# tanwanirahul/surreal

Hardware: AMD Instinct MI355X
Metric: PPO learner env-steps/sec/node (GAE+update) at 1/2/4/8 GPUs; % HBM roofline (higher is better)
Workload: dtype f32; 1 GPU; C3: synthetic PPO learner batch, reference PPO defaults (LSTM 100, horizon 5, heads 300x200, n_step 25, adapt, z-filter, 10/10 epochs), SawyerLift state dims (obs 42, act 8), 1024 segments split over 1 GPU(s) (1024 per GPU); segments_per_gpu=1024, n_step=25, env_steps_per_learn_per_gpu=25600, global_segments=1024, parallelism=single, epochs_run_last=10, ppo_mode=adapt, launch=hipGraph replay

## Files before the change

surreal_amd/csrc/lstm_mfma.hip:

```cpp
#include "smi_device.hpp"
#include "smi_internal.hpp"
#include "lstm_cell.hpp"

namespace smi {

constexpr int LR = 16;
#ifdef SMI_PROF
__device__ unsigned long long g_lstm_ticks[8];
#endif

__host__ __device__ inline int lstm_ld(int k) {
  int l = round4(k);
  if ((l & 7) != 4) l += 4;
  return l;
}

__host__ __device__ inline int lstm_q(int K) { return (((K + 3) >> 2) + 3) & ~3; }

constexpr int MAXUT = 4;
__global__ void __launch_bounds__(kWG)
lstm_fwd_kernel(LstmFwdArgs a) {
  if (a.skip && a.skip[0] != 0) return;
  const int keepS = a.keep > 0 ? a.keep : a.S;
  extern __shared__ __attribute__((aligned(16))) float sm[];
  const int H = a.H, B = a.B, G4 = 4 * H;
  const int LDH = lstm_ld(4 * lstm_q(H));
  float* hA[2] = {sm, sm + LR * LDH};
  const int lane = threadIdx.x & 63, wave = threadIdx.x >> 6;
  const int li = lane & 15, lk = lane >> 4;
  const int r0 = blockIdx.x * LR;
  const int NUT = (H + 15) >> 4;
  const int64_t BH = (int64_t)B * H;
  for (int e = threadIdx.x; e < LR * LDH; e += kWG) {
    const int r = e / LDH, k = e - r * LDH;
    const bool ok = k < H && r0 + r < B;
    const float v = ok ? a.h0[(int64_t)(r0 + r) * H + k] : 0.f;
    hA[0][e] = v;
    hA[1][e] = 0.f;
    if (ok) a.hbuf[(int64_t)(r0 + r) * H + k] = v;
  }
  float creg[MAXUT][4];
#pragma unroll
  for (int u = 0; u < MAXUT; ++u) {
    const int unit = (wave + 4 * u) * 16 + li;
#pragma unroll
    for (int i = 0; i < 4; ++i) {
      const int gr = r0 + lk * 4 + i;
      const bool ok = unit < H && gr < B;
      creg[u][i] = ok ? a.c0[(int64_t)gr * H + unit] : 0.f;
      if (ok && a.cbuf) a.cbuf[(int64_t)gr * H + unit] = creg[u][i];
    }
  }
  const float* wrow[MAXUT][4];
  float bh[MAXUT][4];
#pragma unroll
  for (int u = 0; u < MAXUT; ++u) {
    int unit = (wave + 4 * u) * 16 + li;
    unit = unit < H ? unit : H - 1;
#pragma unroll
    for (int g = 0; g < 4; ++g) {
      wrow[u][g] = a.w_hh + (int64_t)(g * H + unit) * H;
      bh[u][g] = a.b_hh[g * H + unit];
    }
  }
  const int nks = (H + 3) >> 2;
  __syncthreads();
  for (int t = 0; t < a.S; ++t) {
    const float* hp = hA[t & 1];
    float* hn = hA[(t + 1) & 1];
    float xp[MAXUT][4][4];
#pragma unroll
    for (int u = 0; u < MAXUT; ++u) {
      int unit = (wave + 4 * u) * 16 + li;
      unit = unit < H ? unit : H - 1;
#pragma unroll
      for (int i = 0; i < 4; ++i) {
        int gr = r0 + lk * 4 + i;
        gr = gr < B ? gr : B - 1;
        const float* xr = a.xproj + ((int64_t)t * B + gr) * G4 + unit;
#pragma unroll
        for (int g = 0; g < 4; ++g) xp[u][g][i] = xr[g * H];
      }
    }
    f32x4 acc[MAXUT][4];
#pragma unroll
    for (int u = 0; u < MAXUT; ++u)
#pragma unroll
      for (int g = 0; g < 4; ++g) acc[u][g] = f32x4{0.f, 0.f, 0.f, 0.f};
    const float* ap = hp + li * LDH + lk;
    int ks = 0;
    for (; ks + 4 <= nks; ks += 4) {
      float av[4], bv[MAXUT][4][4];
#pragma unroll
      for (int s = 0; s < 4; ++s) {
        const int k = (ks + s) * 4 + lk;
        const int kc = k < H ? k : H - 1;
        av[s] = ap[(ks + s) * 4];
#pragma unroll
        for (int u = 0; u < MAXUT; ++u)
#pragma unroll
          for (int g = 0; g < 4; ++g) bv[u][g][s] = wrow[u][g][kc];
      }
#pragma unroll
      for (int s = 0; s < 4; ++s)
#pragma unroll
        for (int u = 0; u < MAXUT; ++u)
#pragma unroll
          for (int g = 0; g < 4; ++g) acc[u][g] = mfma4(av[s], bv[u][g][s], acc[u][g]);
    }
    for (; ks < nks; ++ks) {
      const int k = ks * 4 + lk;
      const int kc = k < H ? k : H - 1;
      const float av = ap[ks * 4];
#pragma unroll
      for (int u = 0; u < MAXUT; ++u)
#pragma unroll
        for (int g = 0; g < 4; ++g) acc[u][g] = mfma4(av, wrow[u][g][kc], acc[u][g]);
    }
#pragma unroll
    for (int u = 0; u < MAXUT; ++u) {
      const int ut = wave + 4 * u;
      const int unit = ut * 16 + li;
      if (ut >= NUT) continue;
#pragma unroll
      for (int i = 0; i < 4; ++i) {
        const int row = lk * 4 + i, gr = r0 + row;
        const float gi = xp[u][0][i] + (acc[u][0][i] + bh[u][0]);
        const float gf = xp[u][1][i] + (acc[u][1][i] + bh[u][1]);
        const float gg = xp[u][2][i] + (acc[u][2][i] + bh[u][2]);
        const float go = xp[u][3][i] + (acc[u][3][i] + bh[u][3]);
        const float ig = sigm(gi), fg = sigm(gf), cg = ftanh(gg), og = sigm(go);
        const float c = fg * creg[u][i] + ig * cg;
        const float h = og * ftanh(c);
        const bool ok = unit < H && gr < B;
        creg[u][i] = ok ? c : 0.f;
        if (unit < H) hn[row * LDH + unit] = ok ? h : 0.f;
        if (ok) {
          a.hbuf[(int64_t)(t + 1) * BH + (int64_t)gr * H + unit] = h;
          if (a.cbuf && t < keepS) a.cbuf[(int64_t)(t + 1) * BH + (int64_t)gr * H + unit] = c;
          if (a.gates && t < keepS) {
            float* gp = a.gates + ((int64_t)t * B + gr) * G4 + unit;
            gp[0] = ig; gp[H] = fg; gp[2 * H] = cg; gp[3 * H] = og;
          }
        }
      }
    }
    __syncthreads();
  }
}



__global__ void __launch_bounds__(kWG)
lstm_bwd_kernel(LstmBwdArgs a) {
  if (a.skip && a.skip[0] != 0) return;
  extern __shared__ __attribute__((aligned(16))) float sm[];
  const int H = a.H, B = a.B, G4 = 4 * H;
  const int LDG = lstm_ld(G4);
  float* dG[2] = {sm, sm + LR * LDG};
  const int lane = threadIdx.x & 63, wave = threadIdx.x >> 6;
  const int li = lane & 15, lk = lane >> 4;
  const int r0 = blockIdx.x * LR;
  const int NUT = (H + 15) >> 4;
  const int64_t BH = (int64_t)B * H;
  for (int e = threadIdx.x; e < 2 * LR * LDG; e += kWG) sm[e] = 0.f;
  float dcreg[MAXUT][4];
  f32x4 dhrec[MAXUT];
#pragma unroll
  for (int u = 0; u < MAXUT; ++u) {
    dhrec[u] = f32x4{0.f, 0.f, 0.f, 0.f};
#pragma unroll
    for (int i = 0; i < 4; ++i) dcreg[u][i] = 0.f;
  }
  int ucl[MAXUT];
#pragma unroll
  for (int u = 0; u < MAXUT; ++u) {
    const int unit = (wave + 4 * u) * 16 + li;
    ucl[u] = unit < H ? unit : H - 1;
  }
  const int nks = G4 >> 2;
  __syncthreads();
  for (int t = a.S - 1; t >= 0; --t) {
    float* dg = dG[t & 1];
#pragma unroll
    for (int u = 0; u < MAXUT; ++u) {
      const int ut = wave + 4 * u;
      const int unit = ut * 16 + li;
      if (ut >= NUT) continue;
#pragma unroll
      for (int i = 0; i < 4; ++i) {
        const int row = lk * 4 + i;
        int gr = r0 + row;
        const bool ok = unit < H && gr < B;
        gr = gr < B ? gr : B - 1;
        const int uc = ucl[u];
        const float* gp = a.gates + ((int64_t)t * B + gr) * G4 + uc;
        const float ig = gp[0], fg = gp[H], cg = gp[2 * H], og = gp[3 * H];
        const float c = a.cbuf[(int64_t)(t + 1) * BH + (int64_t)gr * H + uc];
        const float cp = a.cbuf[(int64_t)t * BH + (int64_t)gr * H + uc];
        const float dh = a.dh[(int64_t)t * BH + (int64_t)gr * H + uc] + dhrec[u][i];
        const float tc = ftanh(c);
        const float dc = dh * og * (1.f - tc * tc) + dcreg[u][i];
        const float d_o = (dh * tc) * (og * (1.f - og));
        const float d_i = (dc * cg) * (ig * (1.f - ig));
        const float d_g = (dc * ig) * (1.f - cg * cg);
        const float d_f = (dc * cp) * (fg * (1.f - fg));
        dcreg[u][i] = ok ? dc * fg : 0.f;
        if (ok) {
          float* o = a.dgates + ((int64_t)t * B + gr) * G4 + unit;
          o[0] = d_i; o[H] = d_f; o[2 * H] = d_g; o[3 * H] = d_o;
          float* l = dg + row * LDG + unit;
          l[0] = d_i; l[H] = d_f; l[2 * H] = d_g; l[3 * H] = d_o;
        }
      }
    }
    __syncthreads();
    if (t == 0) break;
#pragma unroll
    for (int u = 0; u < MAXUT; ++u) dhrec[u] = f32x4{0.f, 0.f, 0.f, 0.f};
    const float* ap = dg + li * LDG + lk;
    int ks = 0;
    for (; ks + 8 <= nks; ks += 8) {
      float av[8], bv[MAXUT][8];
#pragma unroll
      for (int s = 0; s < 8; ++s) {
        const int k = (ks + s) * 4 + lk;
        av[s] = ap[(ks + s) * 4];
#pragma unroll
        for (int u = 0; u < MAXUT; ++u) bv[u][s] = a.w_hh[(int64_t)k * H + ucl[u]];
      }
#pragma unroll
      for (int s = 0; s < 8; ++s)
#pragma unroll
        for (int u = 0; u < MAXUT; ++u) dhrec[u] = mfma4(av[s], bv[u][s], dhrec[u]);
    }
    for (; ks < nks; ++ks) {
      const int k = ks * 4 + lk;
      const float av = ap[ks * 4];
#pragma unroll
      for (int u = 0; u < MAXUT; ++u) dhrec[u] = mfma4(av, a.w_hh[(int64_t)k * H + ucl[u]], dhrec[u]);
    }
  }
}

constexpr int kWG8 = 512;
template <int N>
__device__ __forceinline__ void load_row(const float* r, int n, float* dst) {
  static_assert(N % 4 == 0, "rows in float4 runs");
  const uintptr_t ad = reinterpret_cast<uintptr_t>(r);
  if ((ad & 15) == 0 && (n & 3) == 0) {
#pragma unroll
    for (int k = 0; k < N; k += 4) {
      const float4 v = k < n ? *reinterpret_cast<const float4*>(r + k) : float4{0.f, 0.f, 0.f, 0.f};
      dst[k] = v.x; dst[k + 1] = v.y; dst[k + 2] = v.z; dst[k + 3] = v.w;
    }
  } else if ((ad & 7) == 0 && (n & 1) == 0) {
#pragma unroll
    for (int k = 0; k < N; k += 2) {
      const float2 v = k < n ? *reinterpret_cast<const float2*>(r + k) : float2{0.f, 0.f};
      dst[k] = v.x; dst[k + 1] = v.y;
    }
  } else {
#pragma unroll
    for (int k = 0; k < N; ++k) dst[k] = k < n ? r[k] : 0.f;
  }
}

constexpr int LR4 = 4;
constexpr int LSTM_HQ = 4;

__device__ __forceinline__ f32x4 mfma4x64(float a, float b, f32x4 c) {
  return __builtin_amdgcn_mfma_f32_4x4x1f32(a, b, c, 4, 0, 0);
}

__device__ __attribute__((aligned(16))) float g_lstm_zero4[4] = {0.f, 0.f, 0.f, 0.f};
template <int N, int V>
__device__ __forceinline__ void load_row_v(const float* r, int n, float* dst) {
  static_assert(N % 4 == 0 && (V == 4 || V == 2), "vector rows");
#pragma unroll
  for (int k = 0; k < N; k += V) {
    const float* src = k < n ? r + k : g_lstm_zero4;
    if constexpr (V == 4) {
      const float4 v = *reinterpret_cast<const float4*>(src);
      dst[k] = v.x; dst[k + 1] = v.y; dst[k + 2] = v.z; dst[k + 3] = v.w;
    } else {
      const float2 v = *reinterpret_cast<const float2*>(src);
      dst[k] = v.x; dst[k + 1] = v.y;
    }
  }
}

template <int N>
__device__ __forceinline__ void load_col(const float* t, int n, int ld, uint32_t zoff, int col,
                                         float* dst) {
#pragma unroll
  for (int k = 0; k < N; ++k) {
    const uint32_t row = k < n ? (uint32_t)(k * ld) : zoff;
    dst[k] = t[row + (uint32_t)col];
  }
}

template <int KP, int KX, bool VF = false, bool IMG = false>
__global__ void __launch_bounds__(kWG8)
lstm_fwd_r4_kernel(LstmFwdArgs a) {
  if (a.skip && a.skip[0] != 0) return;
  LSTM_T0();
  const int keepS = a.keep > 0 ? a.keep : a.S;
  constexpr int KXS = KX > 0 ? KX : 8;
  __shared__ __attribute__((aligned(16))) float hS[2][LR4 * KP];
  __shared__ __attribute__((aligned(16))) float xS[2][LR4 * KXS];
  __shared__ float pre[LR4][4 * KP];
  const int H = a.H, B = a.B, G4 = 4 * H;
  const int tid = threadIdx.x, lane = tid & 63, wave = tid >> 6;
  const int r0 = blockIdx.x * LR4;
  const int64_t BH = (int64_t)B * H;
  const int col = wave * 64 + lane;
  const bool cact = wave * 64 < G4;
  const int colc = col < G4 ? col : G4 - 1;
  float w[KP];
  float wx[KXS];
  float bh = a.b_hh[colc];
  if constexpr (KX > 0) bh += a.b_ih[colc];
  if constexpr (IMG) {
    load_col<KP>(a.w_hh, H, G4, (uint32_t)(H * G4), colc, w);
    if constexpr (KX > 0) load_col<KX>(a.w_ih, a.din, G4, (uint32_t)((a.din + H) * G4), colc, wx);
  } else if constexpr (VF) {
    load_row_v<KP, 4>(a.w_hh + (int64_t)colc * H, H, w);
    if constexpr (KX > 0) load_row_v<KX, 2>(a.w_ih + (int64_t)colc * a.din, a.din, wx);
  } else {
    load_row<KP>(a.w_hh + (int64_t)colc * H, H, w);
    if constexpr (KX > 0) load_row<KX>(a.w_ih + (int64_t)colc * a.din, a.din, wx);
  }
  const int xr = tid / KXS, xk = tid - (tid / KXS) * KXS;
  const bool xown = KX > 0 && tid < LR4 * KXS;
  const int64_t xoff0 = (int64_t)min(r0 + xr, B - 1) * a.ldx + min(xk, a.din - 1);
  const bool xval = xk < a.din;
  auto xload = [&](int t) -> float { return a.x[(int64_t)t * B * a.ldx + xoff0]; };
  float xnext = 0.f, x0 = 0.f;
  if constexpr (KX > 0) {
    x0 = xload(0);
    xnext = xload(a.S > 1 ? 1 : 0);
  }
  const bool cell = tid < LR4 * H;
  const int crow = cell ? tid / H : 0;
  const int cunit = cell ? tid - crow * H : 0;
  const int cgr = r0 + crow;
  const bool cok = cell && cgr < B;
  const float c0v = a.c0[(int64_t)min(cgr, B - 1) * H + cunit];
  static_assert(LR4 * KP <= kWG8, "one h0 slot per thread");
  const int he = min(tid, LR4 * KP - 1);
  const int hr = he / KP, hk = he - hr * KP;
  float h0v = a.h0[(int64_t)min(r0 + hr, B - 1) * H + min(hk, H - 1)];
  asm volatile("" : "+v"(h0v));
  if constexpr (KX > 0) asm volatile("" : "+v"(x0));
  if constexpr (KX > 0) {
    if (xown && a.S > 0) xS[0][xr * KXS + xk] = xval ? x0 : 0.f;
  }
  float creg = cok ? c0v : 0.f;
  if (cok && a.cbuf) a.cbuf[(int64_t)cgr * H + cunit] = creg;
  if (tid < LR4 * KP) {
    const bool ok = hk < H && r0 + hr < B;
    const float v = ok ? h0v : 0.f;
    hS[0][he] = v;
    hS[1][he] = 0.f;
    if (ok) a.hbuf[(int64_t)(r0 + hr) * H + hk] = v;
  }
  int64_t xoff[4];
#pragma unroll
  for (int i = 0; i < 4; ++i) {
    const int gr = r0 + i < B ? r0 + i : B - 1;
    xoff[i] = (int64_t)gr * G4 + colc;
  }
  float xp[4] = {0.f, 0.f, 0.f, 0.f};
  if (KX == 0 && a.S > 0) {
#pragma unroll
    for (int i = 0; i < 4; ++i) xp[i] = a.xproj[xoff[i]];
  }
  __syncthreads();
  LSTM_TICK(6);
  f32x4 acc[8];
#pragma unroll
  for (int j = 0; j < 8; ++j) acc[j] = f32x4{0.f, 0.f, 0.f, 0.f};
  auto x_part = [&](int tt) {
    if constexpr (KX > 0) {
      const float4* xr4 = reinterpret_cast<const float4*>(xS[tt & 1] + (lane & 3) * KXS);
      constexpr int NQX = KX / 4;
      float4 q[LSTM_HQ];
#pragma unroll
      for (int j = 0; j < LSTM_HQ && j < NQX; ++j) q[j] = xr4[j];
#pragma unroll
      for (int j = 0; j < NQX; ++j) {
        const float4 u = q[j % LSTM_HQ];
        const int ab = (j & 1) * 4;
        acc[ab + 0] = mfma4x64(u.x, wx[4 * j + 0], acc[ab + 0]);
        acc[ab + 1] = mfma4x64(u.y, wx[4 * j + 1], acc[ab + 1]);
        acc[ab + 2] = mfma4x64(u.z, wx[4 * j + 2], acc[ab + 2]);
        acc[ab + 3] = mfma4x64(u.w, wx[4 * j + 3], acc[ab + 3]);
        if (j + LSTM_HQ < NQX) q[j % LSTM_HQ] = xr4[j + LSTM_HQ];
      }
      __builtin_amdgcn_sched_group_barrier(0x100, LSTM_HQ < NQX ? LSTM_HQ : NQX, 0);
#pragma unroll
      for (int j = 0; j < NQX; ++j) {
        __builtin_amdgcn_sched_group_barrier(0x008, 4, 0);
        if (j + LSTM_HQ < NQX) __builtin_amdgcn_sched_group_barrier(0x100, 1, 0);
      }
    }
  };
  if (cact && a.S > 0) x_part(0);
  for (int t = 0; t < a.S; ++t) {
    const float* hp = hS[t & 1];
    float* hn = hS[(t + 1) & 1];
    if (cact) {
      const float4* hr = reinterpret_cast<const float4*>(hp + (lane & 3) * KP);
      constexpr int NQ = KP / 4;
      float4 q[LSTM_HQ];
#pragma unroll
      for (int j = 0; j < LSTM_HQ; ++j) q[j] = hr[j];
#pragma unroll
      for (int j = 0; j < NQ; ++j) {
        const float4 u = q[j % LSTM_HQ];
        const int ab = (j & 1) * 4;
        acc[ab + 0] = mfma4x64(u.x, w[4 * j + 0], acc[ab + 0]);
        acc[ab + 1] = mfma4x64(u.y, w[4 * j + 1], acc[ab + 1]);
        acc[ab + 2] = mfma4x64(u.z, w[4 * j + 2], acc[ab + 2]);
        acc[ab + 3] = mfma4x64(u.w, w[4 * j + 3], acc[ab + 3]);
        if (j + LSTM_HQ < NQ) q[j % LSTM_HQ] = hr[j + LSTM_HQ];
      }
      __builtin_amdgcn_sched_group_barrier(0x100, LSTM_HQ, 0);
#pragma unroll
      for (int j = 0; j < NQ; ++j) {
        __builtin_amdgcn_sched_group_barrier(0x008, 4, 0);
        if (j + LSTM_HQ < NQ) __builtin_amdgcn_sched_group_barrier(0x100, 1, 0);
      }
      const f32x4 sum = ((acc[0] + acc[1]) + (acc[2] + acc[3])) +
                        ((acc[4] + acc[5]) + (acc[6] + acc[7]));
      if (col < G4) {
#pragma unroll
        for (int i = 0; i < 4; ++i) pre[i][col] = xp[i] + (sum[i] + bh);
      }
      if (KX == 0 && t + 1 < a.S) {
#pragma unroll
        for (int i = 0; i < 4; ++i) xp[i] = a.xproj[(int64_t)(t + 1) * B * G4 + xoff[i]];
      }
    }
    if constexpr (KX > 0) {
      if (xown && t + 1 < a.S) xS[(t + 1) & 1][xr * KXS + xk] = xval ? xnext : 0.f;
      if (xown && t + 2 < a.S) xnext = xload(t + 2);
    }
    LSTM_TICK(0);
    __syncthreads();
    if (cact) {
#pragma unroll
      for (int j = 0; j < 8; ++j) acc[j] = f32x4{0.f, 0.f, 0.f, 0.f};
      if (t + 1 < a.S) x_part(t + 1);
    }
    if (cell) {
      const float ig = sigm(pre[crow][cunit]), fg = sigm(pre[crow][H + cunit]);
      const float cg = ftanh(pre[crow][2 * H + cunit]), og = sigm(pre[crow][3 * H + cunit]);
      const float c = fg * creg + ig * cg;
      const float h = og * ftanh(c);
      creg = cok ? c : 0.f;
      hn[crow * KP + cunit] = cok ? h : 0.f;
      if (cok) {
        a.hbuf[(int64_t)(t + 1) * BH + (int64_t)cgr * H + cunit] = h;
        if (a.cbuf && t < keepS) a.cbuf[(int64_t)(t + 1) * BH + (int64_t)cgr * H + cunit] = c;
        if (a.gates && t < keepS) {
          float* gp = a.gates + ((int64_t)t * B + cgr) * G4 + cunit;
          gp[0] = ig; gp[H] = fg; gp[2 * H] = cg; gp[3 * H] = og;
        }
      }
    }
    LSTM_TICK(1);
    __syncthreads();
    LSTM_TICK(2);
  }
}

template <int KW>
__global__ void __launch_bounds__(kWG8)
lstm_bwd_r4_kernel(LstmBwdArgs a) {
  if (a.skip && a.skip[0] != 0) return;
  LSTM_T0();
  constexpr int G4P = 4 * 128 + KW;
  __shared__ __attribute__((aligned(16))) float dG[LR4 * G4P];
  __shared__ float red[8][LR4][64];
  const int H = a.H, B = a.B, G4 = 4 * H;
  const int tid = threadIdx.x, lane = tid & 63, wave = tid >> 6;
  const int r0 = blockIdx.x * LR4;
  const int64_t BH = (int64_t)B * H;
  const int NU = (H + 63) >> 6;
  const int WPG = 8 / NU;
  const int kw = (G4 + WPG - 1) / WPG;
  const int ug = wave / WPG, kp = wave - ug * WPG;
  const int k0 = kp * kw;
  const int unit = ug * 64 + lane;
  const int uc = unit < H ? unit : H - 1;
  for (int e = tid; e < LR4 * G4P; e += kWG8) dG[e] = 0.f;
  float w[KW];
#pragma unroll
  for (int j = 0; j < KW; ++j) {
    const int k = k0 + j;
    const bool ok = j < kw && k < G4 && unit < H;
    const float x = a.w_hh[(int64_t)(k < G4 ? k : G4 - 1) * H + uc];
    w[j] = ok ? x : 0.f;
  }
  const bool cell = tid < LR4 * H;
  const int crow = cell ? tid / H : 0;
  const int cunit = cell ? tid - crow * H : 0;
  const int cgr = r0 + crow;
  const bool cok = cell && cgr < B;
  const int64_t grc = cgr < B ? cgr : B - 1;
  const int cug = cunit >> 6, cl = cunit & 63;
  float pg[4], pc = 0.f, pcp = 0.f, pdh = 0.f;
  auto fetch = [&](int t) {
    const float* gp = a.gates + ((int64_t)t * B + grc) * G4 + cunit;
    pg[0] = gp[0]; pg[1] = gp[H]; pg[2] = gp[2 * H]; pg[3] = gp[3 * H];
    pc = a.cbuf[(int64_t)(t + 1) * BH + grc * H + cunit];
    pcp = a.cbuf[(int64_t)t * BH + grc * H + cunit];
    pdh = a.dh[(int64_t)t * BH + grc * H + cunit];
  };
  if (cell && a.S > 0) fetch(a.S - 1);
  float dcreg = 0.f;
  __syncthreads();
  LSTM_TICK(7);
  for (int t = a.S - 1; t >= 0; --t) {
    if (cell) {
      float dhr = 0.f;
      if (t < a.S - 1) {
        for (int p = 0; p < WPG; ++p) dhr += red[cug * WPG + p][crow][cl];
      }
      const float ig = pg[0], fg = pg[1], cg = pg[2], og = pg[3];
      const float dh = pdh + dhr;
      const float tc = ftanh(pc);
      const float dc = dh * og * (1.f - tc * tc) + dcreg;
      const float d_o = (dh * tc) * (og * (1.f - og));
      const float d_i = (dc * cg) * (ig * (1.f - ig));
      const float d_g = (dc * ig) * (1.f - cg * cg);
      const float d_f = (dc * pcp) * (fg * (1.f - fg));
      dcreg = cok ? dc * fg : 0.f;
      float* l = dG + crow * G4P + cunit;
      l[0] = cok ? d_i : 0.f; l[H] = cok ? d_f : 0.f;
      l[2 * H] = cok ? d_g : 0.f; l[3 * H] = cok ? d_o : 0.f;
      if (cok) {
        float* o = a.dgates + ((int64_t)t * B + cgr) * G4 + cunit;
        o[0] = d_i; o[H] = d_f; o[2 * H] = d_g; o[3 * H] = d_o;
      }
      if (t > 0) fetch(t - 1);
    }
    LSTM_TICK(3);
    __syncthreads();
    LSTM_TICK(4);
    if (t == 0) break;
    if (wave < NU * WPG) {
      f32x4 acc[8];
#pragma unroll
      for (int j = 0; j < 8; ++j) acc[j] = f32x4{0.f, 0.f, 0.f, 0.f};
      constexpr int NQ = KW / 4, LQ = 4;
      const float4* dr = reinterpret_cast<const float4*>(dG + (lane & 3) * G4P + k0);
      float4 q[LQ];
#pragma unroll
      for (int j = 0; j < LQ && j < NQ; ++j) q[j] = dr[j];
#pragma unroll
      for (int j = 0; j < NQ; ++j) {
        const float4 u = q[j % LQ];
        if (j + LQ < NQ) q[j % LQ] = dr[j + LQ];
        const int a0 = (j & 1) * 4;
        acc[a0 + 0] = mfma4x64(u.x, w[4 * j + 0], acc[a0 + 0]);
        acc[a0 + 1] = mfma4x64(u.y, w[4 * j + 1], acc[a0 + 1]);
        acc[a0 + 2] = mfma4x64(u.z, w[4 * j + 2], acc[a0 + 2]);
        acc[a0 + 3] = mfma4x64(u.w, w[4 * j + 3], acc[a0 + 3]);
        __builtin_amdgcn_sched_barrier(0);
      }
      const f32x4 sum = ((acc[0] + acc[1]) + (acc[2] + acc[3])) +
                        ((acc[4] + acc[5]) + (acc[6] + acc[7]));
#pragma unroll
      for (int i = 0; i < 4; ++i) red[wave][i][lane] = sum[i];
    }
    LSTM_TICK(5);
    __syncthreads();
  }
}

static int device_cus() {
  static int cus = 0;
  if (!cus) {
    int dev = 0;
    (void)hipGetDevice(&dev);
    if (hipDeviceGetAttribute(&cus, hipDeviceAttributeMultiprocessorCount, dev) != hipSuccess || cus < 1)
      cus = 256;
  }
  return cus;
}
static bool lstm_valu(int B, int H) { return H >= 1 && H <= 128 && B <= device_cus(); }
bool lstm_fwd_image_ok(int B, int H) { return H >= 1 && H <= 128 && B >= 1 && !lstm_valu(B, H); }

__global__ void __launch_bounds__(kWG)
lstm_weight_image_kernel(const float* __restrict__ w_ih, const float* __restrict__ w_hh, int din,
                         int H, float* __restrict__ image) {
  const int G4 = 4 * H, nih = G4 * din, nw = nih + G4 * H;
  const int o = blockIdx.x * kWG + threadIdx.x;
  if (o >= nw + G4) return;
  if (o < nih) {
    const int k = o / G4, col = o - k * G4;
    image[o] = w_ih[col * din + k];
  } else if (o < nw) {
    const int k = (o - nih) / G4, col = (o - nih) - k * G4;
    image[o] = w_hh[col * H + k];
  } else {
    image[o] = 0.f;
  }
}

int launch_lstm_weight_image(const float* w_ih, const float* w_hh, int din, int H, float* image,
                             hipStream_t st) {
  if (H < 1 || H > 128 || din < 1 || din > 4096)
    return set_error(SMI_E_ARG, "lstm_weight_image: H must be in [1, 128], din in [1, 4096]");
  const int n = 4 * H * (din + H + 1);
  hipLaunchKernelGGL(lstm_weight_image_kernel, dim3((n + kWG - 1) / kWG), dim3(kWG), 0, st, w_ih,
                     w_hh, din, H, image);
  return check_launch("lstm_weight_image_kernel");
}

#ifdef SMI_PROF
extern "C" int smi_lstm_phase_ticks(unsigned long long* out ) {
  if (hipMemcpyFromSymbol(out, HIP_SYMBOL(g_lstm_ticks), sizeof(g_lstm_ticks)) != hipSuccess)
    return SMI_E_LAUNCH;
  static const unsigned long long zero[8] = {0, 0, 0, 0, 0, 0, 0, 0};
  return hipMemcpyToSymbol(HIP_SYMBOL(g_lstm_ticks), zero, sizeof(zero)) == hipSuccess ? SMI_OK
                                                                                        : SMI_E_LAUNCH;
}
#endif

int64_t lstm_fwd_lds(int H) { return (int64_t)2 * LR * lstm_ld(4 * lstm_q(H)) * 4; }
int64_t lstm_bwd_lds(int H) { return (int64_t)2 * LR * lstm_ld(4 * H) * 4; }

static bool r4_vf(const LstmFwdArgs& a, bool fused_x) {
  auto al = [](const void* p, uintptr_t m) { return (reinterpret_cast<uintptr_t>(p) & m) == 0; };
  if (a.H % 4 != 0 || !al(a.w_hh, 15)) return false;
  return !fused_x || (a.din % 2 == 0 && a.din >= 2 && al(a.w_ih, 7));
}

int launch_lstm_fwd(const float* xproj, const float* w_hh, const float* b_hh, const float* h0,
                    const float* c0, int S, int B, int H, float* hbuf, float* cbuf, float* gates,
                    hipStream_t st, const int* skip, int keep, bool image) {
  if (B <= 0 || S < 0) return SMI_OK;
  if (H < 1 || H > 256) return set_error(SMI_E_ARG, "lstm: hidden size must be in [1, 256]");
  if (image && !lstm_fwd_image_ok(B, H)) return SMI_E_NOFIT;
  LstmFwdArgs a{xproj, w_hh, b_hh, h0, c0, S, B, H, hbuf, cbuf, gates, skip};
  a.keep = keep;
  const int kslot = ktime_begin(st);
  struct End { int s; hipStream_t st; double f;
               ~End() { ktime_end(s, KT_LSTM_FWD, f, st); } } end_{kslot, st, 8.0 * B * H * (double)H * S};
  if (lstm_valu(B, H)) return check_launch(lstm_v_fwd(a, 0, st));
  if (H <= 128) {
    const dim3 g4((B + LR4 - 1) / LR4);
    const bool vf = r4_vf(a, false);
#define SMI_R4F(KP_)                                                                        \
    do {                                                                                    \
      if (image) {                                                                          \
        hipLaunchKernelGGL((lstm_fwd_r4_kernel<KP_, 0, false, true>), g4, dim3(kWG8), 0,    \
                           st, a);                                                          \
        return check_launch("lstm_fwd_r4_kernel<" #KP_ ",0,img>");                          \
      } else if (vf) {                                                                      \
        hipLaunchKernelGGL((lstm_fwd_r4_kernel<KP_, 0, true>), g4, dim3(kWG8), 0, st, a);   \
        return check_launch("lstm_fwd_r4_kernel<" #KP_ ",0,vf>");                           \
      } else {                                                                              \
        hipLaunchKernelGGL((lstm_fwd_r4_kernel<KP_, 0>), g4, dim3(kWG8), 0, st, a);         \
        return check_launch("lstm_fwd_r4_kernel<" #KP_ ",0>");                              \
      }                                                                                     \
    } while (0)
    if (H <= 32) SMI_R4F(32);
    else if (H <= 64) SMI_R4F(64);
    else if (H <= 104) SMI_R4F(104);
    else SMI_R4F(128);
#undef SMI_R4F
  }
  const size_t lds = (size_t)lstm_fwd_lds(H);
  const dim3 grid((B + LR - 1) / LR);
  allow_lds(lstm_fwd_kernel, lds);
  hipLaunchKernelGGL(lstm_fwd_kernel, grid, dim3(kWG), lds, st, a);
  return check_launch("lstm_fwd_kernel<4>");
}

int launch_lstm_fwd_x(const float* x, int64_t ldx, int din, const float* w_ih, const float* b_ih,
                      const float* w_hh, const float* b_hh, const float* h0, const float* c0,
                      int S, int B, int H, float* hbuf, float* cbuf, float* gates,
                      hipStream_t st, const int* skip, int keep, bool image) {
  if (B <= 0 || S <= 0) return SMI_OK;
  if (!lstm_fwd_x_fuses(din, H)) return SMI_E_NOFIT;
  const bool valu = lstm_valu(B, H);
  if (image && valu) return SMI_E_NOFIT;
  if (image && w_hh != w_ih + (int64_t)4 * H * din)
    return set_error(SMI_E_ARG, "lstm: W_hhT must follow W_ihT in the weight image");
  if (valu && lstm_fwd_v_lds(S, din <= 48 ? 48 : 64, (4 * H + 63) & ~63) > kVxMax)
    return SMI_E_NOFIT;
  LstmFwdArgs a{nullptr, w_hh, b_hh, h0, c0, S, B, H, hbuf, cbuf, gates, skip,
                x, ldx, din, w_ih, b_ih, keep};
  const int kslot = ktime_begin(st);
  struct End { int s; hipStream_t st; double f;
               ~End() { ktime_end(s, KT_LSTM_FWD, f, st); } } end_{
      kslot, st, 8.0 * B * H * (double)(H + din) * S};
  if (valu) return check_launch(lstm_v_fwd(a, din <= 48 ? 48 : 64, st));
  const dim3 g4((B + LR4 - 1) / LR4);
  const bool vf = r4_vf(a, true);
#define SMI_R4X(KP_, KX_)                                                                     \
  do {                                                                                        \
    if (image) {                                                                              \
      hipLaunchKernelGGL((lstm_fwd_r4_kernel<KP_, KX_, false, true>), g4, dim3(kWG8), 0, st,  \
                         a);                                                                  \
      return check_launch("lstm_fwd_r4_kernel<" #KP_ "," #KX_ ",img>");                       \
    } else if (vf) {                                                                          \
      hipLaunchKernelGGL((lstm_fwd_r4_kernel<KP_, KX_, true>), g4, dim3(kWG8), 0, st, a);     \
      return check_launch("lstm_fwd_r4_kernel<" #KP_ "," #KX_ ",vf>");                        \
    } else {                                                                                  \
      hipLaunchKernelGGL((lstm_fwd_r4_kernel<KP_, KX_>), g4, dim3(kWG8), 0, st, a);           \
      return check_launch("lstm_fwd_r4_kernel<" #KP_ "," #KX_ ">");                           \
    }                                                                                         \
  } while (0)
  if (din <= 48) {
    if (H <= 64) SMI_R4X(64, 48);
    else SMI_R4X(104, 48);
  } else {
    if (H <= 64) SMI_R4X(64, 64);
    else SMI_R4X(104, 64);
  }
#undef SMI_R4X
}

int lstm_bwd_q_form(int B, int H, const float* w_hh) {
  if (!lstm_valu(B, H) || !lstm_bwd_q_ok(H, w_hh)) return 0;
  return H <= 64 ? 16 : H <= 100 ? 25 : 32;
}

bool lstm_fwd_x_dual_fits(int B0, int B1, int S, int H, int din) {
  if (din < 1 || din > 64 || H < 1 || H > 104 || B0 <= 0 || B1 <= 0)
    return false;
  if (!lstm_valu(B0 + B1, H)) return false;
  return lstm_fwd_v_lds(S, din <= 48 ? 48 : 64, (4 * H + 63) & ~63) <= kVxMax;
}

int launch_lstm_fwd_x_dual(const LstmFwdArgs& a0, const LstmFwdArgs& a1, hipStream_t st) {
  const int H = a0.H, din = a0.din;
  const int smax = a0.S > a1.S ? a0.S : a1.S;
  if (a0.S <= 0 && a1.S <= 0) return SMI_OK;
  if (a0.S <= 0 || a1.S <= 0) return SMI_E_NOFIT;
  if (a0.H != a1.H || a0.din != a1.din || !lstm_fwd_x_dual_fits(a0.B, a1.B, smax, H, din))
    return SMI_E_NOFIT;
  const int kx = din <= 48 ? 48 : 64;
  const int kslot = ktime_begin(st);
  const char* form = lstm_q_fwd_dual(a0, a1, kx, st);
  ktime_end(kslot, KT_LSTM_FWD,
            8.0 * H * (double)(H + din) * ((double)a0.B * a0.S + (double)a1.B * a1.S), st);
  return check_launch(form);
}

int launch_lstm_bwd(const float* dh, const float* gates, const float* cbuf, const float* w_hh,
                    int S, int B, int H, float* dgates, hipStream_t st, const int* skip) {
  if (B <= 0 || S <= 0) return SMI_OK;
  if (H < 1 || H > 256) return set_error(SMI_E_ARG, "lstm: hidden size must be in [1, 256]");
  LstmBwdArgs a{dh, gates, cbuf, w_hh, S, B, H, dgates, skip};
  const int kslot = ktime_begin(st);
  struct End { int s; hipStream_t st; double f;
               ~End() { ktime_end(s, KT_LSTM_BWD, f, st); } } end_{kslot, st,
                                                                 8.0 * B * H * (double)H * (S - 1)};
  if (lstm_valu(B, H)) return check_launch(lstm_v_bwd(a, st));
  if (H <= 128) {
    const int nu = (H + 63) / 64, wpg = 8 / nu;
    const int kw = (4 * H + wpg - 1) / wpg;
    const dim3 g4((B + LR4 - 1) / LR4);
#define SMI_R4B(KW_)                                                              \
    do {                                                                          \
      hipLaunchKernelGGL(lstm_bwd_r4_kernel<KW_>, g4, dim3(kWG8), 0, st, a);      \
      return check_launch("lstm_bwd_r4_kernel<" #KW_ ">");                        \
    } while (0)
    if (kw <= 32) SMI_R4B(32);
    else if (kw <= 104) SMI_R4B(104);
    else SMI_R4B(128);
#undef SMI_R4B
  }
  const size_t lds = (size_t)lstm_bwd_lds(H);
  if (lds > 160 * 1024) return set_error(SMI_E_NOFIT, "lstm: hidden size too large for LDS");
  const dim3 grid((B + LR - 1) / LR);
  allow_lds(lstm_bwd_kernel, lds);
  hipLaunchKernelGGL(lstm_bwd_kernel, grid, dim3(kWG), lds, st, a);
  return check_launch("lstm_bwd_kernel<4>");
}


}
```

Measured before the change: 4.134 million env-steps/s.

## Software-pipeline LSTM backward: double-buffer fetches, hoist gate factors, raise occupancy

Restructures the LSTM BPTT backward kernel. Per-timestep loads now run two steps ahead in double-buffered register sets, and the gate-derivative factors for the next step are computed during the MFMA phase. The dgates stores are issued in the middle of the MFMA loop, and the loop is unrolled by two. It also adds occupancy hints to launch_bounds, fixes WPG at compile time, zeroes the reduction buffer so the first step needs no branch, and uses a zero row to load weights without predication. The goal is to hide global-memory latency on the serial recurrence critical path, at the cost of more register pressure and more complex control flow.

```diff
diff --git a/surreal_amd/csrc/lstm_mfma.hip b/surreal_amd/csrc/lstm_mfma.hip
--- a/surreal_amd/csrc/lstm_mfma.hip
+++ b/surreal_amd/csrc/lstm_mfma.hip
@@ -476,34 +476,55 @@
   }
 }
 
+struct BpttIn { float ig, fg, cg, og, c, cp, dh; };
+struct BpttFac { float tc, omt, fo, fi, fgg, ff; };
+
+__device__ __forceinline__ BpttFac bptt_factors(const BpttIn& s) {
+#pragma clang fp contract(off)
+  BpttFac f;
+  f.tc = ftanh(s.c);
+  f.omt = fmaf(-f.tc, f.tc, 1.f);
+  f.fo = s.og * (1.f - s.og);
+  f.fi = s.ig * (1.f - s.ig);
+  f.fgg = fmaf(-s.cg, s.cg, 1.f);
+  f.ff = s.fg * (1.f - s.fg);
+  return f;
+}
+
+__device__ __forceinline__ float bptt_cell(const BpttIn& s, const BpttFac& f, float dhr, float dcreg,
+                                           float d[4]) {
+#pragma clang fp contract(off)
+  const float dh = s.dh + dhr;
+  const float dc = fmaf(dh * s.og, f.omt, dcreg);
+  d[3] = (dh * f.tc) * f.fo;
+  d[0] = (dc * s.cg) * f.fi;
+  d[2] = (dc * s.ig) * f.fgg;
+  d[1] = (dc * s.cp) * f.ff;
+  return dc * s.fg;
+}
+
+__device__ float g_lstm_zero_row[128];
 template <int KW>
-__global__ void __launch_bounds__(kWG8)
+__global__ void __launch_bounds__(kWG8, KW <= 32 ? 4 : 2)
 lstm_bwd_r4_kernel(LstmBwdArgs a) {
   if (a.skip && a.skip[0] != 0) return;
   LSTM_T0();
   constexpr int G4P = 4 * 128 + KW;
+  constexpr int WPG = KW <= 32 ? 8 : 4;
   __shared__ __attribute__((aligned(16))) float dG[LR4 * G4P];
   __shared__ float red[8][LR4][64];
   const int H = a.H, B = a.B, G4 = 4 * H;
-  const int tid = threadIdx.x, lane = tid & 63, wave = tid >> 6;
+  const int tid = threadIdx.x, lane = tid & 63;
+  const int wave = __builtin_amdgcn_readfirstlane(tid >> 6);
   const int r0 = blockIdx.x * LR4;
-  const int64_t BH = (int64_t)B * H;
-  const int NU = (H + 63) >> 6;
-  const int WPG = 8 / NU;
+  const int64_t BH = (int64_t)B * H, BG4 = (int64_t)B * G4;
   const int kw = (G4 + WPG - 1) / WPG;
   const int ug = wave / WPG, kp = wave - ug * WPG;
   const int k0 = kp * kw;
   const int unit = ug * 64 + lane;
   const int uc = unit < H ? unit : H - 1;
   for (int e = tid; e < LR4 * G4P; e += kWG8) dG[e] = 0.f;
-  float w[KW];
-#pragma unroll
-  for (int j = 0; j < KW; ++j) {
-    const int k = k0 + j;
-    const bool ok = j < kw && k < G4 && unit < H;
-    const float x = a.w_hh[(int64_t)(k < G4 ? k : G4 - 1) * H + uc];
-    w[j] = ok ? x : 0.f;
-  }
+  for (int e = tid; e < 8 * LR4 * 64; e += kWG8) (&red[0][0][0])[e] = 0.f;
   const bool cell = tid < LR4 * H;
   const int crow = cell ? tid / H : 0;
   const int cunit = cell ? tid - crow * H : 0;
@@ -511,74 +532,110 @@
   const bool cok = cell && cgr < B;
   const int64_t grc = cgr < B ? cgr : B - 1;
   const int cug = cunit >> 6, cl = cunit & 63;
-  float pg[4], pc = 0.f, pcp = 0.f, pdh = 0.f;
-  auto fetch = [&](int t) {
-    const float* gp = a.gates + ((int64_t)t * B + grc) * G4 + cunit;
-    pg[0] = gp[0]; pg[1] = gp[H]; pg[2] = gp[2 * H]; pg[3] = gp[3 * H];
-    pc = a.cbuf[(int64_t)(t + 1) * BH + grc * H + cunit];
-    pcp = a.cbuf[(int64_t)t * BH + grc * H + cunit];
-    pdh = a.dh[(int64_t)t * BH + grc * H + cunit];
+  const int64_t goff = grc * G4 + cunit, hoff = grc * H + cunit;
+  auto fetch = [&](int t, BpttIn& s) {
+    const float* gp = a.gates + ((int64_t)t * BG4 + goff);
+    s.ig = gp[0]; s.fg = gp[H]; s.cg = gp[2 * H]; s.og = gp[3 * H];
+    const int64_t o = (int64_t)t * BH + hoff;
+    s.c = a.cbuf[o + BH];
+    s.cp = a.cbuf[o];
+    s.dh = a.dh[o];
   };
-  if (cell && a.S > 0) fetch(a.S - 1);
+  BpttIn sa, sb;
+  fetch(a.S - 1, sa);
+  fetch(a.S > 1 ? a.S - 2 : 0, sb);
+  float w[KW];
+  const int jn = min(kw, G4 - k0);
+#pragma unroll
+  for (int j = 0; j < KW; ++j) {
+    const bool in = j < jn;
+    const float* base = in ? a.w_hh : g_lstm_zero_row;
+    const uint32_t ro = in ? (uint32_t)((k0 + j) * H) : 0u;
+    w[j] = base[ro + (uint32_t)uc];
+  }
+  asm volatile("" : "+v"(sa.ig), "+v"(sa.fg), "+v"(sa.cg), "+v"(sa.og), "+v"(sa.c), "+v"(sa.cp),
+               "+v"(sa.dh));
+  asm volatile("" : "+v"(sb.ig), "+v"(sb.fg), "+v"(sb.cg), "+v"(sb.og), "+v"(sb.c), "+v"(sb.cp),
+               "+v"(sb.dh));
+  BpttFac f = bptt_factors(sa);
   float dcreg = 0.f;
+  __builtin_amdgcn_s_waitcnt(0x0F70);
   __syncthreads();
   LSTM_TICK(7);
-  for (int t = a.S - 1; t >= 0; --t) {
+  auto cells = [&](const BpttIn& x, float d[4]) __attribute__((always_inline)) {
     if (cell) {
+      float r[WPG];
+#pragma unroll
+      for (int p = 0; p < WPG; ++p) r[p] = red[cug * WPG + p][crow][cl];
       float dhr = 0.f;
-      if (t < a.S - 1) {
-        for (int p = 0; p < WPG; ++p) dhr += red[cug * WPG + p][crow][cl];
-      }
-      const float ig = pg[0], fg = pg[1], cg = pg[2], og = pg[3];
-      const float dh = pdh + dhr;
-      const float tc = ftanh(pc);
-      const float dc = dh * og * (1.f - tc * tc) + dcreg;
-      const float d_o = (dh * tc) * (og * (1.f - og));
-      const float d_i = (dc * cg) * (ig * (1.f - ig));
-      const float d_g = (dc * ig) * (1.f - cg * cg);
-      const float d_f = (dc * pcp) * (fg * (1.f - fg));
-      dcreg = cok ? dc * fg : 0.f;
+#pragma unroll
+      for (int p = 0; p < WPG; ++p) dhr += r[p];
+      const float dcf = bptt_cell(x, f, dhr, dcreg, d);
+      dcreg = cok ? dcf : 0.f;
       float* l = dG + crow * G4P + cunit;
-      l[0] = cok ? d_i : 0.f; l[H] = cok ? d_f : 0.f;
-      l[2 * H] = cok ? d_g : 0.f; l[3 * H] = cok ? d_o : 0.f;
-      if (cok) {
-        float* o = a.dgates + ((int64_t)t * B + cgr) * G4 + cunit;
-        o[0] = d_i; o[H] = d_f; o[2 * H] = d_g; o[3 * H] = d_o;
-      }
-      if (t > 0) fetch(t - 1);
+      l[0] = cok ? d[0] : 0.f; l[H] = cok ? d[1] : 0.f;
+      l[2 * H] = cok ? d[2] : 0.f; l[3 * H] = cok ? d[3] : 0.f;
     }
     LSTM_TICK(3);
     __syncthreads();
     LSTM_TICK(4);
-    if (t == 0) break;
-    if (wave < NU * WPG) {
-      f32x4 acc[8];
-#pragma unroll
-      for (int j = 0; j < 8; ++j) acc[j] = f32x4{0.f, 0.f, 0.f, 0.f};
-      constexpr int NQ = KW / 4, LQ = 4;
-      const float4* dr = reinterpret_cast<const float4*>(dG + (lane & 3) * G4P + k0);
-      float4 q[LQ];
-#pragma unroll
-      for (int j = 0; j < LQ && j < NQ; ++j) q[j] = dr[j];
-#pragma unroll
-      for (int j = 0; j < NQ; ++j) {
-        const float4 u = q[j % LQ];
-        if (j + LQ < NQ) q[j % LQ] = dr[j + LQ];
-        const int a0 = (j & 1) * 4;
-        acc[a0 + 0] = mfma4x64(u.x, w[4 * j + 0], acc[a0 + 0]);
-        acc[a0 + 1] = mfma4x64(u.y, w[4 * j + 1], acc[a0 + 1]);
-        acc[a0 + 2] = mfma4x64(u.z, w[4 * j + 2], acc[a0 + 2]);
-        acc[a0 + 3] = mfma4x64(u.w, w[4 * j + 3], acc[a0 + 3]);
-        __builtin_amdgcn_sched_barrier(0);
-      }
-      const f32x4 sum = ((acc[0] + acc[1]) + (acc[2] + acc[3])) +
-                        ((acc[4] + acc[5]) + (acc[6] + acc[7]));
-#pragma unroll
-      for (int i = 0; i < 4; ++i) red[wave][i][lane] = sum[i];
-    }
+  };
+  auto store = [&](int t, const float d[4]) __attribute__((always_inline)) {
+    if (cok) {
+      float* o = a.dgates + ((int64_t)t * BG4 + (int64_t)cgr * G4 + cunit);
+      o[0] = d[0]; o[H] = d[1]; o[2 * H] = d[2]; o[3 * H] = d[3];
+    }
+  };
+  auto step = [&](int t, BpttIn& x, BpttIn& y) __attribute__((always_inline)) {
+    float d[4] = {0.f, 0.f, 0.f, 0.f};
+    cells(x, d);
+    f32x4 acc[8];
+#pragma unroll
+    for (int j = 0; j < 8; ++j) acc[j] = f32x4{0.f, 0.f, 0.f, 0.f};
+    constexpr int NQ = KW / 4, LQ = 4;
+    const float4* dr = reinterpret_cast<const float4*>(dG + (lane & 3) * G4P + k0);
+    float4 q[LQ];
+#pragma unroll
+    for (int j = 0; j < LQ && j < NQ; ++j) q[j] = dr[j];
+#pragma unroll
+    for (int j = 0; j < NQ; ++j) {
+      const float4 u = q[j % LQ];
+      if (j + LQ < NQ) q[j % LQ] = dr[j + LQ];
+      const int a0 = (j & 1) * 4;
+      acc[a0 + 0] = mfma4x64(u.x, w[4 * j + 0], acc[a0 + 0]);
+      acc[a0 + 1] = mfma4x64(u.y, w[4 * j + 1], acc[a0 + 1]);
+      acc[a0 + 2] = mfma4x64(u.z, w[4 * j + 2], acc[a0 + 2]);
+      acc[a0 + 3] = mfma4x64(u.w, w[4 * j + 3], acc[a0 + 3]);
+      if (j == 1) {
+        store(t, d);
+        fetch(t > 1 ? t - 2 : 0, x);
+      }
+      __builtin_amdgcn_sched_barrier(0);
+    }
+    asm volatile("" : "+v"(y.ig), "+v"(y.fg), "+v"(y.cg), "+v"(y.og), "+v"(y.c), "+v"(y.cp),
+                 "+v"(y.dh));
+    f = bptt_factors(y);
+    asm volatile("" : "+v"(f.tc), "+v"(f.omt), "+v"(f.fo), "+v"(f.fi), "+v"(f.fgg), "+v"(f.ff));
+    const f32x4 sum = ((acc[0] + acc[1]) + (acc[2] + acc[3])) +
+                      ((acc[4] + acc[5]) + (acc[6] + acc[7]));
+#pragma unroll
+    for (int i = 0; i < 4; ++i) red[wave][i][lane] = sum[i];
     LSTM_TICK(5);
     __syncthreads();
-  }
+  };
+  int t = a.S - 1;
+  for (int i = t >> 1; i > 0; --i, t -= 2) {
+    step(t, sa, sb);
+    step(t - 1, sb, sa);
+  }
+  float d[4] = {0.f, 0.f, 0.f, 0.f};
+  if (t == 1) {
+    step(1, sa, sb);
+    cells(sb, d);
+  } else {
+    cells(sa, d);
+  }
+  store(0, d);
 }
 
 static int device_cus() {
```

Result: faster. 4.217 million env-steps/s (median of 6 runs) (+2.0%).
